# ecmwf/anemoi-core

Measured on AMD Instinct MI355X. Metric: forward nodes*channels/sec on O96 GraphTransformer, higher is better.
Workload: dtype bf16; 1 GPU; AnemoiModelEncProcDec forward, O96 data grid (40320 nodes, 84 vars x 2 steps) -> icosphere res 5 hidden mesh (10242 nodes, 81840 edges), GraphTransformer processor 16 layers x 512 ch x 16 heads, enc 62912 / dec 120960 edges, batch 1; parallelism=single GPU, hip_graph=True, graph_equals_eager=True, graph_segments=1

## Files before the change

### anemoi_core_amd/_lib.py

```python
from __future__ import annotations

import ctypes as C
import os
import threading

ABI_VERSION = 17
LIB_PATH = os.path.join(os.path.dirname(os.path.abspath(__file__)), "lib", "libanemoi_hip.so")

F32, BF16, F16 = 0, 1, 2
ACT_NONE, ACT_GELU = 0, 1
E_INVALID, E_UNSUPPORTED, E_LAUNCH = -1, -2, -3

_p, _i64, _i32, _f = C.c_void_p, C.c_int64, C.c_int32, C.c_float



class LinearPlan(C.Structure):
    _fields_ = [(name, _i32) for name in ("kernel", "tile_m", "tile_n", "pingpong", "stage_k", "mi", "wr", "kg", "stages", "epi", "main_rows",
                                          "tail_rows", "ln_tail_begin")]


SIGNATURES = {
    "anemoi_hip_abi_version": ([], C.c_int),
    "anemoi_hip_last_error": ([], C.c_char_p),
# ... 39 lines not shown
    "anemoi_edge_ln_residual_segment_sum_fwd": ([_p, _i64, _p, _i64, _p, _p, _f, _p, _p, _i64, _p, _i64, _i32, _i32, C.c_int, _p], C.c_int),
    "anemoi_segment_sum_rows": ([_p, _i64, _p, _p, _p, _i64, _i32, _i32, C.c_int, _p], C.c_int),
    "anemoi_gather_add_rows": ([_p, _i64, _p, _i64, _p, _p, _i64, _i32, _i32, C.c_int, _p], C.c_int),
    "anemoi_transpose_pad": ([_p, _i64, _p, _i64, _i32, _i32, _i32, C.c_int, _p], C.c_int),
    "anemoi_glu_fwd": ([_p, _i64, _p, _i64, _i32, _i32, _i32, C.c_int, _p], C.c_int),
    "anemoi_glu_bwd": ([_p, _i64, _p, _i64, _p, _i64, _i32, _i32, _i32, C.c_int, _p], C.c_int),
    "anemoi_gather_rows": ([_p, _i64, _p, _p, _i64, _i32, _i32, C.c_int, _p], C.c_int),
    "anemoi_peer_alloc": ([C.POINTER(_p), _i64, _i32], C.c_int),
    "anemoi_peer_free": ([_p], C.c_int),
    "anemoi_peer_export": ([_p, _p], C.c_int),
    "anemoi_peer_open": ([_p, C.POINTER(_p)], C.c_int),
    "anemoi_peer_close": ([_p], C.c_int),
    "anemoi_gt_chain_rows_per_tile": ([_i32], C.c_int),
    "anemoi_gt_chain2_fwd": ([_p, C.c_int, _p], C.c_int),
    "anemoi_gt_rowchain_fwd": ([_p, C.c_int, _p], C.c_int),
    "anemoi_gt_cluster_chain_fwd": ([_p, C.c_int, _p], C.c_int),
    "anemoi_gt_cluster_chain_workspace_bytes": ([], _i64),
    "anemoi_gnn_edge_chain_fwd": ([_p, _i64, _p, _i64, _p, _p, _i64, _p, _p, _p, _p, _p, _p, _p, _p, _p, _f, _p, _i64, _i32, _i32, C.c_int, _p], C.c_int),
    "anemoi_gnn_mlp_chain_fwd": ([_p, _i64, _i32, _p, _p, _p, _p, _p, _p, _p, _p, _f, _p, _i64, _p, _i64, _i32, _i32, C.c_int, _p], C.c_int),
    "anemoi_gnn_node_chain_segsum_fwd": ([_p, _i64, _p, _i64, _p, _p, _p, _p, _p, _p, _p, _p, _p, _f, _p, _i64, _p, _p, _i32, _p, _i64, _i32, _i32,
                                          C.c_int, _p], C.c_int),
    "anemoi_gnn_node_chain_fwd": ([_p, _i64, _p, _i64, _p, _p, _p, _p, _p, _p, _p, _p, _f, _p, _i64, _p, _p, _i32, _p, _i64, _i32, _i32, C.c_int, _p], C.c_int),
    "anemoi_peer_exchange_rows": ([_p, _i64, _p, _p, _i32, _i32, _i32, _p, _p, _i64, _p], C.c_int),
    "anemoi_window_attention_fwd": ([_p, _i64, _p, _i64, _p, _i64, _p, _i64, _p, _i32, _i32, _i32, _i32, _i32, _f, _f, _p, C.c_int, _p], C.c_int),
    "anemoi_sparse_project_fwd": ([_p, _i64, _i64, _i32, _i64, _i32, _i32, _p, _p, _p, _p, _p, _p, _p, _i64, _i64, _i32, _i32, _i32, C.c_int, C.c_int, _p], C.c_int),
}


EXPERIMENT_SIGNATURES = {
    "anemoi_gt_chain_fwd": ([_p, C.c_int, _p], C.c_int),
# ... 57 lines not shown
```

### anemoi_core_amd/csrc/chain2_core.h

```cpp
#pragma once
#include "chain_core.h"

namespace anemoi {

template <typename T>
__device__ __forceinline__ void gemm128(const unsigned char* abuf, int lane, frag8 (&ring)[2][8], const char* cur, int64_t cs, const char* nxt,
                                        int64_t ns, uint32_t loff, f32x4 (&acc)[3][8], int nq = 8) {
  asm volatile("" : "+v"(lane));
  const int x = lane & 15, ks = lane >> 4;
  const unsigned char* arow = abuf + x * kRowBytes;
  frag8 fa[3];
#pragma unroll
  for (int mi = 0; mi < 3; ++mi) fa[mi] = *reinterpret_cast<const frag8*>(arow + mi * 16 * kRowBytes + ((ks ^ x) << 4));
  const int last = 2 * nq - 1;
#pragma unroll 1
  for (int q = 0; q < nq; ++q) {
    const char* p0 = q < nq - 1 ? cur + (q + 1) * 8192 : nxt;
    const char* p1 = q < nq - 1 ? cur + cs + (q + 1) * 8192 : nxt + ns;
#pragma unroll
    for (int j = 0; j < 2; ++j) {
      const int st = q * 2 + j;
      const int sn = st < last ? st + 1 : last;
      frag8 fn[3];
#pragma unroll
// ... 2 lines not shown
      const gptr_t g0 = uniform_ptr(p0 + j * 4096), g1 = uniform_ptr(p1 + j * 4096);
#pragma unroll
      for (int ni = 0; ni < 8; ++ni) {
#pragma unroll
        for (int mi = 0; mi < 3; ++mi) acc[mi][ni] = cmfma<T>(ring[j][ni], fa[mi], acc[mi][ni]);
        ring[j][ni] = *reinterpret_cast<gfrag_t>((ni < 4 ? g0 : g1) + loff + (ni & 3) * 1024);
        __builtin_amdgcn_sched_barrier(0);
      }
#pragma unroll
      for (int mi = 0; mi < 3; ++mi) fa[mi] = fn[mi];
      __builtin_amdgcn_sched_barrier(0);
    }
  }
}

template <typename T>
__device__ __forceinline__ void gemm64(const unsigned char* abuf, int lane, frag8 (&ring)[2][8], const char* cur, const char* nxt, int64_t ns,
                                       uint32_t loff, f32x4 (&acc)[3][8], int ng = 4) {
  asm volatile("" : "+v"(lane));
  const int x = lane & 15, ks = lane >> 4;
  const unsigned char* arow = abuf + x * kRowBytes;
  frag8 fa[3];
#pragma unroll
  for (int mi = 0; mi < 3; ++mi) fa[mi] = *reinterpret_cast<const frag8*>(arow + mi * 16 * kRowBytes + ((ks ^ x) << 4));
  const int last = ng * 4 - 1;
#pragma unroll 1
  for (int q = 0; q < ng; ++q) {
#pragma unroll
    for (int j = 0; j < 4; ++j) {
      const int st = q * 4 + j;
      const int sn = st < last ? st + 1 : last;
      frag8 fn[3];
#pragma unroll
      for (int mi = 0; mi < 3; ++mi) fn[mi] = *reinterpret_cast<const frag8*>(arow + mi * 16 * kRowBytes + (((sn * 4 + ks) ^ x) << 4));
      __builtin_amdgcn_sched_barrier(0);
      const char* pf = q < ng - 1 ? cur + (q + 1) * 16384 + j * 4096 : (j < 2 ? nxt + j * 4096 : nxt + ns + (j - 2) * 4096);
      const gptr_t g0 = uniform_ptr(pf);
#pragma unroll
      for (int ni = 0; ni < 4; ++ni) {
#pragma unroll
        for (int mi = 0; mi < 3; ++mi) acc[mi][ni] = cmfma<T>(ring[j & 1][(j >> 1) * 4 + ni], fa[mi], acc[mi][ni]);
        ring[j & 1][(j >> 1) * 4 + ni] = *reinterpret_cast<gfrag_t>(g0 + loff + ni * 1024);
        __builtin_amdgcn_sched_barrier(0);
      }
#pragma unroll
      for (int mi = 0; mi < 3; ++mi) fa[mi] = fn[mi];
      __builtin_amdgcn_sched_barrier(0);
    }
  }
}
__device__ __forceinline__ void ring_prologue64(frag8 (&ring)[2][8], const char* f0, uint32_t loff) {
#pragma unroll
  for (int j = 0; j < 4; ++j) {
    const gptr_t g0 = uniform_ptr(f0 + j * 4096);
#pragma unroll
    for (int ni = 0; ni < 4; ++ni) {
      ring[j & 1][(j >> 1) * 4 + ni] = *reinterpret_cast<gfrag_t>(g0 + loff + ni * 1024);
      __builtin_amdgcn_sched_barrier(0);
    }
  }
}
// ... 75 lines not shown
```

### anemoi_core_amd/csrc/chain_core.h

```cpp
#pragma once
#include "common.h"

namespace anemoi {

using frag8 = __attribute__((ext_vector_type(8))) short;
using f32x4 = __attribute__((ext_vector_type(4))) float;

template <typename T>
__device__ __forceinline__ f32x4 cmfma(frag8 a, frag8 b, f32x4 c);
template <>
__device__ __forceinline__ f32x4 cmfma<bf16_t>(frag8 a, frag8 b, f32x4 c) {
  using bf8 = __attribute__((ext_vector_type(8))) __bf16;
  return __builtin_amdgcn_mfma_f32_16x16x32_bf16(__builtin_bit_cast(bf8, a), __builtin_bit_cast(bf8, b), c, 0, 0, 0);
}
template <>
__device__ __forceinline__ f32x4 cmfma<f16_t>(frag8 a, frag8 b, f32x4 c) {
  using h8 = __attribute__((ext_vector_type(8))) _Float16;
  return __builtin_amdgcn_mfma_f32_16x16x32_f16(__builtin_bit_cast(h8, a), __builtin_bit_cast(h8, b), c, 0, 0, 0);
}

using u32x2 = __attribute__((ext_vector_type(2))) unsigned int;
using u32x4 = __attribute__((ext_vector_type(4))) unsigned int;

template <typename T>
// ... 91 lines not shown
#pragma unroll
      for (int mi = 0; mi < NB; ++mi) fa[mi] = fn[mi];
      __builtin_amdgcn_sched_barrier(0);
    }
  }
  if (flip >= 0) __builtin_amdgcn_s_setprio(0);
}

__device__ __forceinline__ void lds_barrier() {
  asm volatile("s_waitcnt lgkmcnt(0)" ::: "memory");
  __builtin_amdgcn_s_barrier();
  asm volatile("" ::: "memory");
}

__device__ __forceinline__ int panel_off(int row, int slot16) { return row * kRowBytes + ((slot16 ^ (row & 15)) << 4); }
template <typename B>
__device__ __forceinline__ B* panel_at(B* buf, int row, int slot16) { return buf + row * kRowBytes + ((slot16 ^ (row & 15)) << 4); }
template <int NI>
constexpr int kWaves = kCh / (16 * NI);

#ifndef ANEMOI_CHAIN2_NT
#define ANEMOI_CHAIN2_NT 1
#endif
__device__ __forceinline__ u32x4 stream_load(const u32x4* p) {
  if constexpr ((ANEMOI_CHAIN2_NT & 1) != 0) return __builtin_nontemporal_load(p);
  else return *p;
}
__device__ __forceinline__ void stream_store(u32x4 v, u32x4* p) {
  if constexpr ((ANEMOI_CHAIN2_NT & 2) != 0) __builtin_nontemporal_store(v, p);
  else if constexpr ((ANEMOI_CHAIN2_NT & 4) != 0) asm volatile("global_store_dwordx4 %0, %1, off sc1" ::"v"(p), "v"(v) : "memory");
  else *p = v;
}
// ... 108 lines not shown
    for (int ni = 0; ni < 4; ++ni)
      *reinterpret_cast<u32x2*>(strip + m * 128 + (((ni * 2 + (lc.g >> 1)) ^ ((m >> 1) & 7)) << 4) + (lc.g & 1) * 8) = pk[mi][ni];
  }
  asm volatile("s_waitcnt lgkmcnt(0)" ::: "memory");
  const int rl = (lc.g << 1) | (lc.x >> 3), sl = lc.x & 7;
#pragma unroll
  for (int it = 0; it < 2 * NB; ++it) {
    const int m = it * 8 + rl;
    const u32x4 v = *reinterpret_cast<const u32x4*>(strip + m * 128 + ((sl ^ ((m >> 1) & 7)) << 4));
    if (m < nr) *reinterpret_cast<u32x4*>(out + (int64_t)m * ld + sl * 8) = v;
  }
  asm volatile("s_waitcnt lgkmcnt(0)" ::: "memory");
}


template <typename T, int NI, bool ROWS>
__device__ __forceinline__ void init_acc(f32x4 (&acc)[3][8], const unsigned char* vec, int col0, const unsigned char* rows, int lane, int w) {
  const LaneCols<NI> lc = lane_cols<NI>(lane, w);
#pragma unroll
  for (int ni = 0; ni < NI; ++ni) {
    float b[4];
    unpack4<T>(*reinterpret_cast<const u32x2*>(vec + (col0 + w * (16 * NI) + ni * 16 + lc.g * 4) * 2), b);
#pragma unroll
    for (int mi = 0; mi < 3; ++mi) {
      if (ROWS) {
        float r[4];
        unpack4<T>(*reinterpret_cast<const u32x2*>(rows + (mi * 16 + lc.x) * kRowBytes + lc.coff[ni]), r);
        acc[mi][ni] = f32x4{b[0] + r[0], b[1] + r[1], b[2] + r[2], b[3] + r[3]};
      } else {
        acc[mi][ni] = f32x4{b[0], b[1], b[2], b[3]};
      }
    }
  }
}

enum class Add { None, Bias, BiasRows };
template <typename T, int NI, Add ADD, bool STATS, bool STORE = true>
__device__ __forceinline__ void round_rows(f32x4 (&acc)[3][8], unsigned char* dst, float* red, int lane, int w, const unsigned char* vec = nullptr, int col0 = 0) {
  const LaneCols<NI> lc = lane_cols<NI>(lane, w);
  u32x2 rb[NI], rr[NI];
  if constexpr (ADD == Add::Bias) {
#pragma unroll
    for (int ni = 0; ni < NI; ++ni) rb[ni] = *reinterpret_cast<const u32x2*>(vec + (col0 + w * (16 * NI) + ni * 16 + lc.g * 4) * 2);
  }
#pragma unroll
  for (int mi = 0; mi < 3; ++mi) {
    unsigned char* drow = dst + (mi * 16 + lc.x) * kRowBytes;
    if constexpr (ADD == Add::BiasRows) {
#pragma unroll
      for (int h = 0; h < NI / 4; ++h) {
#pragma unroll
        for (int ni = 4 * h; ni < 4 * h + 4; ++ni) {
          rb[ni] = *reinterpret_cast<const u32x2*>(vec + (col0 + w * (16 * NI) + ni * 16 + lc.g * 4) * 2);
          rr[ni] = *reinterpret_cast<const u32x2*>(drow + lc.coff[ni]);
        }
        __builtin_amdgcn_sched_barrier(0);
      }
    }
#pragma unroll
    for (int ni = 0; ni < NI; ++ni) {
      float o[4] = {acc[mi][ni][0], acc[mi][ni][1], acc[mi][ni][2], acc[mi][ni][3]};
      if constexpr (ADD != Add::None) {
// ... 28 lines not shown
  const LaneCols<NI> lc = lane_cols<NI>(lane, w);
#pragma unroll
  for (int mi = 0; mi < 3; ++mi) {
    unsigned char* drow = dst + (mi * 16 + lc.x) * kRowBytes;
#pragma unroll
    for (int ni = 0; ni < NI; ++ni) {
      float o[4] = {acc[mi][ni][0], acc[mi][ni][1], acc[mi][ni][2], acc[mi][ni][3]};
      gelu_fast2(o[0], o[1]);
      gelu_fast2(o[2], o[3]);
      *reinterpret_cast<u32x2*>(drow + lc.coff[ni]) = pack4<T>(o);
      if (ni & 1) __builtin_amdgcn_sched_barrier(0);
    }
  }
}

template <typename T, int NI>
__device__ __forceinline__ void normalise_rows(const f32x4 (&acc)[3][8], const float* red, float eps, unsigned char* dst, int lane, int w) {
  const LaneCols<NI> lc = lane_cols<NI>(lane, w);
#pragma unroll
  for (int mi = 0; mi < 3; ++mi) {
    float mu, rstd;
    merge_partials<kWaves<NI>>(red, mi * 16 + lc.x, eps, mu, rstd);
    const float nm = -mu * rstd;
    unsigned char* drow = dst + (mi * 16 + lc.x) * kRowBytes;
#pragma unroll
    for (int ni = 0; ni < NI; ++ni) {
      float o[4];
#pragma unroll
      for (int r = 0; r < 4; ++r) o[r] = fmaf(acc[mi][ni][r], rstd, nm);
      *reinterpret_cast<u32x2*>(drow + lc.coff[ni]) = pack4<T>(o);
    }
  }
}
template <typename T, int NI>
__device__ __forceinline__ void normalise_regs(f32x4 (&acc)[3][8], const float* red, float eps, int lane, int w) {
  const LaneCols<NI> lc = lane_cols<NI>(lane, w);
#pragma unroll
  for (int mi = 0; mi < 3; ++mi) {
    float mu, rstd;
    merge_partials<kWaves<NI>>(red, mi * 16 + lc.x, eps, mu, rstd);
    const float nm = -mu * rstd;
#pragma unroll
    for (int ni = 0; ni < NI; ++ni)
#pragma unroll
      for (int r = 0; r < 4; ++r) acc[mi][ni][r] = fmaf(acc[mi][ni][r], rstd, nm);
  }
}

template <typename T, int NI>
__device__ __forceinline__ void store_staged(const unsigned char* strip, T* out, int64_t ld, int nr, int lane, int w) {
  asm volatile("s_waitcnt lgkmcnt(0)" ::: "memory");
  asm volatile("" : "+v"(lane), "+s"(w));
  constexpr int kLpr = 2 * NI, kRpi = 64 / kLpr;
  const int rl = lane >> (NI == 8 ? 4 : 3), sl = lane & (kLpr - 1);
#pragma unroll
  for (int it = 0; it < kPanel / kRpi; ++it) {
    const int row = it * kRpi + rl;
    const u32x4 v = *reinterpret_cast<const u32x4*>(panel_at(strip, row, w * kLpr + sl));
    if (row < nr) stream_store(v, reinterpret_cast<u32x4*>(out + (int64_t)row * ld + w * (16 * NI) + sl * 8));
  }
}

}
```

### anemoi_core_amd/csrc/gt_rowchain.hip

```cpp
#include "chain2_core.h"

namespace anemoi {

struct RowChainArgs {
  const void* x;   int64_t ld_x;  int k_in;
  const char* we;  int ng;
  const char* wq;  int qc;
  const void* vec;
  float eps;
  void* xout;      int64_t ld_out;
  void* qout;      int64_t ld_q;
  int n_rows, rows_per_tile, n_tiles;
};
constexpr int kRcVecOff = vec_off(8);
constexpr int kRcVecMax = 2560;
constexpr int kRowChainSmem = kRcVecOff + kRcVecMax * 2;
static_assert(kRowChainSmem <= 160 * 1024, "LDS budget");

struct XRows {
  u32x4 v[6];
  __device__ __forceinline__ void request(const void* x, int64_t ld, int k_in, int ng, int r0, int nr, int tid, int es) {
    const int spr = 16 * ng, n = kPanel * spr, kin16 = k_in >> 3;
#pragma unroll
    for (int k = 0; k < 6; ++k) {
      const int i = tid + 512 * k;
      if (k * 512 < n) {
        const int row = min(i / spr, kPanel - 1), slot = i % spr;
        const bool live = row < nr && slot < kin16 && i < n;
        const unsigned char* p = reinterpret_cast<const unsigned char*>(x) + ((int64_t)(r0 + min(row, nr - 1)) * ld + min(slot, kin16 - 1) * 8) * es;
        const u32x4 t = stream_load(reinterpret_cast<const u32x4*>(p));
        v[k] = live ? t : u32x4{0u, 0u, 0u, 0u};
      }
    }
  }
  __device__ __forceinline__ void store(unsigned char* buf, int ng, int tid) {
    const int spr = 16 * ng, n = kPanel * spr;
#pragma unroll
    for (int k = 0; k < 6; ++k) {
      const int i = tid + 512 * k;
      if (i < n) {
        const int row = i / spr, slot = i % spr;
        *reinterpret_cast<u32x4*>(panel_at(buf, row, slot)) = v[k];
      }
    }
  }
};

template <typename T>
__global__ __launch_bounds__(512, 1) void gt_rowchain_kernel(RowChainArgs a) {
  extern __shared__ __attribute__((aligned(16))) unsigned char smem[];
  unsigned char* const bufA = smem;
  unsigned char* const bufB = smem + kBufBytes;
  unsigned char* const bufC = smem + 2 * kBufBytes;
  float* const red = reinterpret_cast<float*>(smem + kRedOff);
  const unsigned char* const vec = smem + kRcVecOff;
  const int tid = threadIdx.x, lane = tid & 63;
  const int w8 = __builtin_amdgcn_readfirstlane(tid >> 6), wq = w8 & 3, grp = w8 >> 2;
  const uint32_t loff = lane * 16;
  const int qc = a.qc, ng = a.ng;
  const int64_t se = (int64_t)ng * 16384;
  const char* const wes = a.we + (int64_t)w8 * se;
// ... 186 lines not shown
  const int w8 = __builtin_amdgcn_readfirstlane(tid >> 6);
  c.wq = w8 & 3;
  c.loff = c.lane * 16;
  c.b0 = (int)blockIdx.x;
  c.grid = (int)gridDim.x;
  if (c.b0 >= a.n_tiles) return;
  c.n = (a.n_tiles - c.b0 + c.grid - 1) / c.grid;
  {
    const int n16 = (512 + 512 * a.qc) / 8;
    if (tid < n16) reinterpret_cast<u32x4*>(smem + kRc2Vec)[tid] = reinterpret_cast<const u32x4*>(a.vec)[tid];
  }
  if (w8 < 4) pipe_role_a<T>(a, c, smem);
  else pipe_role_b<T>(a, c, smem);
}

template <typename T>
static int launch_rowchain(const RowChainArgs& a, hipStream_t st) {
  static PerDeviceOnce once;
  once.run([&] { (void)hipFuncSetAttribute(reinterpret_cast<const void*>(&gt_rowchain_kernel<T>), hipFuncAttributeMaxDynamicSharedMemorySize, kRowChainSmem); });
  int grid = a.n_tiles < 256 ? a.n_tiles : 256;
  if (a.n_tiles > 256) {
    const int rounds = (a.n_tiles + 255) / 256;
    grid = (a.n_tiles + rounds - 1) / rounds;
  }
  if (a.n_tiles > grid && a.k_in <= 256) {
    static PerDeviceOnce once2;
    once2.run([&] { (void)hipFuncSetAttribute(reinterpret_cast<const void*>(&gt_rowchain_pipe_kernel<T>), hipFuncAttributeMaxDynamicSharedMemorySize, kRowChain2Smem); });
    hipLaunchKernelGGL((gt_rowchain_pipe_kernel<T>), dim3(grid), dim3(512), kRowChain2Smem, st, a);
    return check_launch("gt_rowchain_pipe_kernel");
  }
  hipLaunchKernelGGL((gt_rowchain_kernel<T>), dim3(grid), dim3(512), kRowChainSmem, st, a);
  return check_launch("gt_rowchain_kernel");
}

}

using namespace anemoi;

extern "C" int anemoi_gt_rowchain_fwd(const anemoi_gt_rowchain_args_t* p, anemoi_dtype_t dtype, void* stream) {
  ANEMOI_REQUIRE(p != nullptr, "gt_rowchain_fwd: null argument block");
  ANEMOI_REQUIRE(dtype == ANEMOI_BF16 || dtype == ANEMOI_F16, "gt_rowchain_fwd: 16-bit model dtypes only");
  ANEMOI_REQUIRE(p->n_rows >= 0 && p->channels == kCh, "gt_rowchain_fwd: channels=%d (this kernel is built for %d)", p->channels, kCh);
  if (p->n_rows == 0) return ANEMOI_OK;
  ANEMOI_REQUIRE(p->in_features > 0 && p->in_features <= kCh && p->in_features % 8 == 0,
                 "gt_rowchain_fwd: in_features=%d must be a multiple of 8 up to %d (rows move as 16-byte pieces)", p->in_features, kCh);
  ANEMOI_REQUIRE(p->q_out_features > 0 && p->q_out_features % kCh == 0 && p->q_out_features <= 4 * kCh,
                 "gt_rowchain_fwd: q_out_features=%d must be a multiple of %d up to %d", p->q_out_features, kCh, 4 * kCh);
  ANEMOI_REQUIRE(p->x && p->we && p->wq && p->vec && p->q_out, "gt_rowchain_fwd: null operand");
  const auto al16 = [](const void* q) { return (reinterpret_cast<uintptr_t>(q) & 15) == 0; };
  ANEMOI_REQUIRE(al16(p->x) && al16(p->we) && al16(p->wq) && al16(p->vec) && al16(p->x_out) && al16(p->q_out), "gt_rowchain_fwd: operands must be 16-byte aligned");
  ANEMOI_REQUIRE(p->ld_x >= p->in_features && p->ld_x % 8 == 0 && p->ld_q >= p->q_out_features && p->ld_q % 8 == 0 &&
                     (p->x_out == nullptr || (p->ld_out >= kCh && p->ld_out % 8 == 0)),
                 "gt_rowchain_fwd: leading dimensions too small or not multiples of 8 elements");
  RowChainArgs a{};
  a.x = p->x; a.ld_x = p->ld_x; a.k_in = p->in_features;
  a.we = (const char*)p->we; a.ng = (p->in_features + 127) / 128;
  a.wq = (const char*)p->wq; a.qc = p->q_out_features / kCh;
  a.vec = p->vec;
  a.eps = p->ln_eps;
  a.xout = p->x_out; a.ld_out = p->ld_out;
  a.qout = p->q_out; a.ld_q = p->ld_q;
  a.n_rows = p->n_rows;
  a.rows_per_tile = p->rows_per_tile > 0 ? p->rows_per_tile : kPanel;
  ANEMOI_REQUIRE(a.rows_per_tile <= kPanel, "gt_rowchain_fwd: rows_per_tile=%d exceeds the %d-row panel", a.rows_per_tile, kPanel);
  a.n_tiles = (a.n_rows + a.rows_per_tile - 1) / a.rows_per_tile;
  hipStream_t st = as_stream(stream);
  return dtype == ANEMOI_BF16 ? launch_rowchain<bf16_t>(a, st) : launch_rowchain<f16_t>(a, st);
}
```

### anemoi_core_amd/layers/mapper.py

```python
from __future__ import annotations

import os
from typing import Optional

import torch
from torch import Tensor, nn

from .. import ops
from ..distributed import primitives as comm
from ..distributed.partition import (
    build_graph_partition_from_shard_info,
    ensure_edges_are_dst_sorted,
    local_bipartite_graph,
    shard_edges_1hop,
)
from ..distributed.shapes import BipartiteGraphShardInfo, comm_rank, comm_size, get_shard_sizes, model_is_distributed
from .block import GraphConvMapperBlock, GraphTransformerMapperBlock
from .handoff import Carrier, inference_in, plain_layer_norm
from .kernels import PaddedLinear
from .mlp import MLP
from .utils import compute_mlp_hidden_dim, load_layer_kernels
from ..utils.tensors import version


_ROW_CHAIN = os.environ.get("ANEMOI_ROW_CHAIN", "1") != "0"
_ROW_CHAIN_MIN_ROWS = int(os.environ.get("ANEMOI_ROW_CHAIN_MIN_ROWS", "4096"))
_TAIL_PROJ = os.environ.get("ANEMOI_TAIL_PROJ", "1") != "0"
_ROW_CHAIN_GEMM_BAND = tuple(int(v) for v in os.environ.get("ANEMOI_ROW_CHAIN_GEMM_BAND", "16384:262144").split(":"))


class _LocalGraphCache:

    def __init__(self, keep: int = 4):
        self.entries: dict = {}
        self.keep = keep

    def get(self, key, build):
        hit = self.entries.get(key)
        if hit is None:
            hit = build()
            if len(self.entries) >= self.keep:
                self.entries.pop(next(iter(self.entries)))
            self.entries[key] = hit
# ... 61 lines not shown
        self.shard_strategy = shard_strategy
        self.proc = GraphTransformerMapperBlock(
            in_channels=hidden_dim, hidden_dim=compute_mlp_hidden_dim(hidden_dim, mlp_hidden_ratio), out_channels=hidden_dim,
            attn_channels=attn_channels, num_heads=num_heads, edge_dim=edge_dim, qk_norm=qk_norm,
            mlp_implementation=mlp_implementation, layer_kernels=self.layer_factory, shard_strategy=shard_strategy,
            graph_attention_backend=graph_attention_backend, edge_pre_mlp=edge_pre_mlp,
        )
        self.emb_nodes_dst = self.layer_factory.Linear(self.in_channels_dst, self.hidden_dim)
        self._emb_src, self._emb_dst = PaddedLinear(), PaddedLinear()

    def _tail_projection(self):
        return None

    def _row_chain_ok(self, x: Tensor, lin, ln, projs: list) -> bool:
        return (_ROW_CHAIN and x.is_cuda and x.dim() == 2 and x.dtype != torch.float32 and x.shape[0] >= _ROW_CHAIN_MIN_ROWS
                and not (_ROW_CHAIN_GEMM_BAND[0] < x.shape[0] < _ROW_CHAIN_GEMM_BAND[1])
                and self.hidden_dim == ops.CHAIN_CHANNELS and plain_layer_norm(ln) and lin.in_features <= x.shape[1] and lin.bias is not None
                and ops.gt_row_chain_supported(x, sum(p.out_features for p in projs)) and all(p.in_features == ops.CHAIN_CHANNELS for p in projs)
                and inference_in(x, lin, ln, *projs))

    def _row_chain(self, x: Tensor, lin, side: str, want_x: bool):
        blk = self.proc
        ln = blk.layer_norm_attention_src if side == "src" else blk.layer_norm_attention_dest
        projs = [blk.lin_key, blk.lin_value] if side == "src" else [blk.lin_query, blk.lin_self]
        if not self._row_chain_ok(x, lin, ln, projs):
            return None
        params = [lin.weight, lin.bias, ln.weight, ln.bias] + [q for m in projs for q in (m.weight, m.bias)]
        K = x.shape[1]

        def build():
            w = lin.weight if lin.in_features == K else torch.nn.functional.pad(lin.weight, (0, K - lin.in_features))
            wq = torch.cat([m.weight for m in projs], dim=0)
            bq = torch.cat([m.bias if m.bias is not None else m.weight.new_zeros(m.out_features) for m in projs])
            wqg, dq = ops.fold_layer_norm(wq, bq, ln.weight, ln.bias)
            return ops.pack_embedding_frag(w), ops.pack_weight_frag(wqg), torch.cat([lin.bias.float(), dq]).to(x.dtype).contiguous(), wq.shape[0]

        we, wqg, vec, q_out = blk._fused.derived(f"rowchain:{side}:{K}", params, build)
        return ops.gt_row_chain(x, we, wqg, vec, q_out, ln.eps, want_x_out=want_x)

    def _embed(self, padded: PaddedLinear, x: Tensor, lin, side: str, carrier: Optional[Carrier]) -> Tensor:
        ln = self.proc.layer_norm_attention_src if side == "src" else self.proc.layer_norm_attention_dest
        if carrier is not None:
            r = self._row_chain(x, lin, side, want_x=side == "dst" or self.proc.update_src_nodes)
            if r is not None:
                y, proj = r
                return carrier.put(y if y is not None else x.new_empty((x.shape[0], 0)), proj=proj)
            if self.proc._ln_fold_ok(ln, x):
                y, stats = padded.with_row_stats(x, lin)
                return y if stats is None else carrier.put(y, stats=stats)
        return padded(x, lin)

    @comm.scoped_forward
    def forward(self, x, batch_size: int, shard_info: BipartiteGraphShardInfo, edge_attr: Tensor, edge_index: Tensor,
# ... 223 lines not shown
```

### anemoi_core_amd/ops.py

```python
from __future__ import annotations

from dataclasses import dataclass
from typing import NamedTuple, Optional

import os

import torch
from torch import Tensor

from . import _ext, _lib

_DT = {torch.float32: _lib.F32, torch.bfloat16: _lib.BF16, torch.float16: _lib.F16}


def _dt(t: Tensor) -> int:
    try:
        return _DT[t.dtype]
    except KeyError:
        raise ValueError(f"unsupported dtype {t.dtype}; supported: float32, bfloat16, float16") from None


try:
    _raw_stream = torch._C._cuda_getCurrentRawStream
except AttributeError:
# ... 1005 lines not shown
                ("x_out", _p), ("ld_out", _i64), ("q_out", _p), ("ld_q", _i64), ("n_rows", _i32), ("channels", _i32), ("rows_per_tile", _i32)]


def pack_embedding_frag(weight: Tensor) -> Tensor:
    O, K = weight.shape
    pad = (-K) % 128
    w = weight.detach()
    return pack_weight_frag(torch.nn.functional.pad(w, (0, pad)) if pad else w)


def gt_row_chain_supported(x: Tensor, q_out: int) -> bool:
    return (x.is_cuda and x.dim() == 2 and x.dtype in (torch.bfloat16, torch.float16) and 0 < x.shape[1] <= CHAIN_CHANNELS and x.shape[1] % 8 == 0
            and x.stride(1) == 1 and x.stride(0) % 8 == 0 and q_out > 0 and q_out % CHAIN_CHANNELS == 0 and q_out <= 4 * CHAIN_CHANNELS)


def gt_row_chain(x: Tensor, we: Tensor, wqg: Tensor, vec: Tensor, q_out_features: int, ln_eps: float, *, want_x_out: bool = True,
                 rows_per_tile: int = 0):
    _dev(x, we, wqg, vec)
    N, K = x.shape
    dt, D = x.dtype, CHAIN_CHANNELS
    if not gt_row_chain_supported(x, q_out_features):
        raise NotImplementedError(f"gt_row_chain: x {tuple(x.shape)} {dt} / q_out={q_out_features} (16-bit rows of <= {D} columns, a multiple of 8; q_out a multiple of {D})")
    kp = (K + 127) // 128 * 128
    for name, w, numel in (("we", we, D * kp), ("wqg", wqg, q_out_features * D)):
        if w.dim() != 1 or w.numel() != numel or w.dtype != dt or not w.is_contiguous():
            raise ValueError(f"gt_row_chain: {name} must be the contiguous fragment-major image ({numel} x {dt})")
    if vec.dim() != 1 or vec.numel() != D + q_out_features or vec.dtype != dt or not vec.is_contiguous():
        raise ValueError(f"gt_row_chain: vec must be contiguous [{D + q_out_features}] {dt} = cat[be, dq]")
    x_out = torch.empty((N, D), dtype=dt, device=x.device) if want_x_out else None
    q_out = torch.empty((N, q_out_features), dtype=dt, device=x.device)
# ... 271 lines not shown
```

### include/anemoi_hip.h

```cpp
#ifndef ANEMOI_HIP_H
#define ANEMOI_HIP_H

#include <stdint.h>

#ifdef __cplusplus
extern "C" {
#endif

#define ANEMOI_HIP_ABI_VERSION 17

typedef enum { ANEMOI_F32 = 0, ANEMOI_BF16 = 1, ANEMOI_F16 = 2 } anemoi_dtype_t;
typedef enum { ANEMOI_ACT_NONE = 0, ANEMOI_ACT_GELU = 1 } anemoi_act_t;

#define ANEMOI_OK 0
#define ANEMOI_E_INVALID (-1)
#define ANEMOI_E_UNSUPPORTED (-2)
#define ANEMOI_E_LAUNCH (-3)

int anemoi_hip_abi_version(void);
const char* anemoi_hip_last_error(void);

int anemoi_gt_attention_fwd(const void* q, int64_t ldq, const void* k, int64_t ldk, const void* v, int64_t ldv,
                            const void* e, int64_t lde, const int32_t* row, const int32_t* colptr,
                            const void* addend, int64_t ldadd, void* out, int64_t ldo, float* lse,
// ... 175 lines not shown
} anemoi_gt_chain2_args_t;
int anemoi_gt_chain2_fwd(const anemoi_gt_chain2_args_t* args, anemoi_dtype_t dtype, void* stream);
int anemoi_gt_chain_rows_per_tile(int32_t n_rows);

typedef struct anemoi_gt_rowchain_args {
  const void* x;      int64_t ld_x;       int32_t in_features;
  const void* we;
  const void* wq;     int32_t q_out_features;
  const void* vec;
  float ln_eps;
  void* x_out;        int64_t ld_out;
  void* q_out;        int64_t ld_q;
  int32_t n_rows;     int32_t channels;   int32_t rows_per_tile;
} anemoi_gt_rowchain_args_t;
int anemoi_gt_rowchain_fwd(const anemoi_gt_rowchain_args_t* args, anemoi_dtype_t dtype, void* stream);

typedef struct anemoi_gt_cluster_chain_args {
  const void* attn;   int64_t ld_attn;
  const void* x_res;  int64_t ld_x;
  const void* wp;
  const void* w1;     int32_t hidden;
  const void* w2;
  const void* wq;     int32_t q_out_features;
  const void* vec;
  float ln1_eps;      float lnq_eps;
  const void* extra;  int64_t ld_extra;
  void* x_out;        int64_t ld_out;
  void* q_out;        int64_t ld_q;
  void* ln_out;       int64_t ld_ln;
  void* q_out2;       int64_t ld_q2;      int32_t q_split;
// ... 40 lines not shown
```

Measured before the change: 8.635 billion nodes*channels/s.

## Add 96-row tall tile variant of the row-chain embed kernel for narrow inputs

```diff
diff --git a/anemoi_core_amd/_lib.py b/anemoi_core_amd/_lib.py
--- a/anemoi_core_amd/_lib.py
+++ b/anemoi_core_amd/_lib.py
@@ -77,6 +77,7 @@
     "anemoi_gt_chain_rows_per_tile": ([_i32], C.c_int),
     "anemoi_gt_chain2_fwd": ([_p, C.c_int, _p], C.c_int),
     "anemoi_gt_rowchain_fwd": ([_p, C.c_int, _p], C.c_int),
+    "anemoi_gt_rowchain_rows_per_tile": ([_i32, _i32], C.c_int),
     "anemoi_gt_cluster_chain_fwd": ([_p, C.c_int, _p], C.c_int),
     "anemoi_gt_cluster_chain_workspace_bytes": ([], _i64),
     "anemoi_gnn_edge_chain_fwd": ([_p, _i64, _p, _i64, _p, _p, _i64, _p, _p, _p, _p, _p, _p, _p, _p, _p, _f, _p, _i64, _i32, _i32, C.c_int, _p], C.c_int),
diff --git a/anemoi_core_amd/csrc/chain2_core.h b/anemoi_core_amd/csrc/chain2_core.h
--- a/anemoi_core_amd/csrc/chain2_core.h
+++ b/anemoi_core_amd/csrc/chain2_core.h
@@ -40,15 +40,15 @@
   }
 }
 
-template <typename T>
+template <typename T, int NB = 3, int ROWB = kRowBytes>
 __device__ __forceinline__ void gemm64(const unsigned char* abuf, int lane, frag8 (&ring)[2][8], const char* cur, const char* nxt, int64_t ns,
-                                       uint32_t loff, f32x4 (&acc)[3][8], int ng = 4) {
+                                       uint32_t loff, f32x4 (&acc)[NB][8], int ng = 4) {
   asm volatile("" : "+v"(lane));
   const int x = lane & 15, ks = lane >> 4;
-  const unsigned char* arow = abuf + x * kRowBytes;
-  frag8 fa[3];
+  const unsigned char* arow = abuf + x * ROWB;
+  frag8 fa[NB];
 #pragma unroll
-  for (int mi = 0; mi < 3; ++mi) fa[mi] = *reinterpret_cast<const frag8*>(arow + mi * 16 * kRowBytes + ((ks ^ x) << 4));
+  for (int mi = 0; mi < NB; ++mi) fa[mi] = *reinterpret_cast<const frag8*>(arow + mi * 16 * ROWB + ((ks ^ x) << 4));
   const int last = ng * 4 - 1;
 #pragma unroll 1
   for (int q = 0; q < ng; ++q) {
@@ -56,21 +56,21 @@
     for (int j = 0; j < 4; ++j) {
       const int st = q * 4 + j;
       const int sn = st < last ? st + 1 : last;
-      frag8 fn[3];
+      frag8 fn[NB];
 #pragma unroll
-      for (int mi = 0; mi < 3; ++mi) fn[mi] = *reinterpret_cast<const frag8*>(arow + mi * 16 * kRowBytes + (((sn * 4 + ks) ^ x) << 4));
+      for (int mi = 0; mi < NB; ++mi) fn[mi] = *reinterpret_cast<const frag8*>(arow + mi * 16 * ROWB + (((sn * 4 + ks) ^ x) << 4));
       __builtin_amdgcn_sched_barrier(0);
       const char* pf = q < ng - 1 ? cur + (q + 1) * 16384 + j * 4096 : (j < 2 ? nxt + j * 4096 : nxt + ns + (j - 2) * 4096);
       const gptr_t g0 = uniform_ptr(pf);
 #pragma unroll
       for (int ni = 0; ni < 4; ++ni) {
 #pragma unroll
-        for (int mi = 0; mi < 3; ++mi) acc[mi][ni] = cmfma<T>(ring[j & 1][(j >> 1) * 4 + ni], fa[mi], acc[mi][ni]);
+        for (int mi = 0; mi < NB; ++mi) acc[mi][ni] = cmfma<T>(ring[j & 1][(j >> 1) * 4 + ni], fa[mi], acc[mi][ni]);
         ring[j & 1][(j >> 1) * 4 + ni] = *reinterpret_cast<gfrag_t>(g0 + loff + ni * 1024);
         __builtin_amdgcn_sched_barrier(0);
       }
 #pragma unroll
-      for (int mi = 0; mi < 3; ++mi) fa[mi] = fn[mi];
+      for (int mi = 0; mi < NB; ++mi) fa[mi] = fn[mi];
       __builtin_amdgcn_sched_barrier(0);
     }
   }
diff --git a/anemoi_core_amd/csrc/chain_core.h b/anemoi_core_amd/csrc/chain_core.h
--- a/anemoi_core_amd/csrc/chain_core.h
+++ b/anemoi_core_amd/csrc/chain_core.h
@@ -129,8 +129,8 @@
 }
 
 __device__ __forceinline__ int panel_off(int row, int slot16) { return row * kRowBytes + ((slot16 ^ (row & 15)) << 4); }
-template <typename B>
-__device__ __forceinline__ B* panel_at(B* buf, int row, int slot16) { return buf + row * kRowBytes + ((slot16 ^ (row & 15)) << 4); }
+template <int ROWB = kRowBytes, typename B>
+__device__ __forceinline__ B* panel_at(B* buf, int row, int slot16) { return buf + row * ROWB + ((slot16 ^ (row & 15)) << 4); }
 template <int NI>
 constexpr int kWaves = kCh / (16 * NI);
 
@@ -269,18 +269,18 @@
 }
 
 
-template <typename T, int NI, bool ROWS>
-__device__ __forceinline__ void init_acc(f32x4 (&acc)[3][8], const unsigned char* vec, int col0, const unsigned char* rows, int lane, int w) {
+template <typename T, int NI, bool ROWS, int NB = 3, int ROWB = kRowBytes>
+__device__ __forceinline__ void init_acc(f32x4 (&acc)[NB][8], const unsigned char* vec, int col0, const unsigned char* rows, int lane, int w) {
   const LaneCols<NI> lc = lane_cols<NI>(lane, w);
 #pragma unroll
   for (int ni = 0; ni < NI; ++ni) {
     float b[4];
     unpack4<T>(*reinterpret_cast<const u32x2*>(vec + (col0 + w * (16 * NI) + ni * 16 + lc.g * 4) * 2), b);
 #pragma unroll
-    for (int mi = 0; mi < 3; ++mi) {
+    for (int mi = 0; mi < NB; ++mi) {
       if (ROWS) {
         float r[4];
-        unpack4<T>(*reinterpret_cast<const u32x2*>(rows + (mi * 16 + lc.x) * kRowBytes + lc.coff[ni]), r);
+        unpack4<T>(*reinterpret_cast<const u32x2*>(rows + (mi * 16 + lc.x) * ROWB + lc.coff[ni]), r);
         acc[mi][ni] = f32x4{b[0] + r[0], b[1] + r[1], b[2] + r[2], b[3] + r[3]};
       } else {
         acc[mi][ni] = f32x4{b[0], b[1], b[2], b[3]};
@@ -290,8 +290,8 @@
 }
 
 enum class Add { None, Bias, BiasRows };
-template <typename T, int NI, Add ADD, bool STATS, bool STORE = true>
-__device__ __forceinline__ void round_rows(f32x4 (&acc)[3][8], unsigned char* dst, float* red, int lane, int w, const unsigned char* vec = nullptr, int col0 = 0) {
+template <typename T, int NI, Add ADD, bool STATS, bool STORE = true, int NB = 3, int ROWB = kRowBytes>
+__device__ __forceinline__ void round_rows(f32x4 (&acc)[NB][8], unsigned char* dst, float* red, int lane, int w, const unsigned char* vec = nullptr, int col0 = 0) {
   const LaneCols<NI> lc = lane_cols<NI>(lane, w);
   u32x2 rb[NI], rr[NI];
   if constexpr (ADD == Add::Bias) {
@@ -299,8 +299,8 @@
     for (int ni = 0; ni < NI; ++ni) rb[ni] = *reinterpret_cast<const u32x2*>(vec + (col0 + w * (16 * NI) + ni * 16 + lc.g * 4) * 2);
   }
 #pragma unroll
-  for (int mi = 0; mi < 3; ++mi) {
-    unsigned char* drow = dst + (mi * 16 + lc.x) * kRowBytes;
+  for (int mi = 0; mi < NB; ++mi) {
+    unsigned char* drow = dst + (mi * 16 + lc.x) * ROWB;
     if constexpr (ADD == Add::BiasRows) {
 #pragma unroll
       for (int h = 0; h < NI / 4; ++h) {
@@ -359,32 +359,32 @@
   }
 }
 
+template <typename T, int NI, int NB = 3, int ROWB = kRowBytes>
+__device__ __forceinline__ void normalise_rows(const f32x4 (&acc)[NB][8], const float* red, float eps, unsigned char* dst, int lane, int w) {
+  const LaneCols<NI> lc = lane_cols<NI>(lane, w);
+#pragma unroll
+  for (int mi = 0; mi < NB; ++mi) {
+    float mu, rstd;
+    merge_partials<kWaves<NI>>(red, mi * 16 + lc.x, eps, mu, rstd);
+    const float nm = -mu * rstd;
+    unsigned char* drow = dst + (mi * 16 + lc.x) * ROWB;
+#pragma unroll
+    for (int ni = 0; ni < NI; ++ni) {
+      float o[4];
+#pragma unroll
+      for (int r = 0; r < 4; ++r) o[r] = fmaf(acc[mi][ni][r], rstd, nm);
+      *reinterpret_cast<u32x2*>(drow + lc.coff[ni]) = pack4<T>(o);
+    }
+  }
+}
 template <typename T, int NI>
-__device__ __forceinline__ void normalise_rows(const f32x4 (&acc)[3][8], const float* red, float eps, unsigned char* dst, int lane, int w) {
+__device__ __forceinline__ void normalise_regs(f32x4 (&acc)[3][8], const float* red, float eps, int lane, int w) {
   const LaneCols<NI> lc = lane_cols<NI>(lane, w);
 #pragma unroll
   for (int mi = 0; mi < 3; ++mi) {
     float mu, rstd;
     merge_partials<kWaves<NI>>(red, mi * 16 + lc.x, eps, mu, rstd);
     const float nm = -mu * rstd;
-    unsigned char* drow = dst + (mi * 16 + lc.x) * kRowBytes;
-#pragma unroll
-    for (int ni = 0; ni < NI; ++ni) {
-      float o[4];
-#pragma unroll
-      for (int r = 0; r < 4; ++r) o[r] = fmaf(acc[mi][ni][r], rstd, nm);
-      *reinterpret_cast<u32x2*>(drow + lc.coff[ni]) = pack4<T>(o);
-    }
-  }
-}
-template <typename T, int NI>
-__device__ __forceinline__ void normalise_regs(f32x4 (&acc)[3][8], const float* red, float eps, int lane, int w) {
-  const LaneCols<NI> lc = lane_cols<NI>(lane, w);
-#pragma unroll
-  for (int mi = 0; mi < 3; ++mi) {
-    float mu, rstd;
-    merge_partials<kWaves<NI>>(red, mi * 16 + lc.x, eps, mu, rstd);
-    const float nm = -mu * rstd;
 #pragma unroll
     for (int ni = 0; ni < NI; ++ni)
 #pragma unroll
@@ -392,16 +392,16 @@
   }
 }
 
-template <typename T, int NI>
+template <typename T, int NI, int NB = 3, int ROWB = kRowBytes>
 __device__ __forceinline__ void store_staged(const unsigned char* strip, T* out, int64_t ld, int nr, int lane, int w) {
   asm volatile("s_waitcnt lgkmcnt(0)" ::: "memory");
   asm volatile("" : "+v"(lane), "+s"(w));
   constexpr int kLpr = 2 * NI, kRpi = 64 / kLpr;
   const int rl = lane >> (NI == 8 ? 4 : 3), sl = lane & (kLpr - 1);
 #pragma unroll
-  for (int it = 0; it < kPanel / kRpi; ++it) {
+  for (int it = 0; it < 16 * NB / kRpi; ++it) {
     const int row = it * kRpi + rl;
-    const u32x4 v = *reinterpret_cast<const u32x4*>(panel_at(strip, row, w * kLpr + sl));
+    const u32x4 v = *reinterpret_cast<const u32x4*>(panel_at<ROWB>(strip, row, w * kLpr + sl));
     if (row < nr) stream_store(v, reinterpret_cast<u32x4*>(out + (int64_t)row * ld + w * (16 * NI) + sl * 8));
   }
 }
diff --git a/anemoi_core_amd/csrc/gt_rowchain.hip b/anemoi_core_amd/csrc/gt_rowchain.hip
--- a/anemoi_core_amd/csrc/gt_rowchain.hip
+++ b/anemoi_core_amd/csrc/gt_rowchain.hip
@@ -17,15 +17,16 @@
 constexpr int kRowChainSmem = kRcVecOff + kRcVecMax * 2;
 static_assert(kRowChainSmem <= 160 * 1024, "LDS budget");
 
-struct XRows {
+template <int ROWS = kPanel, int ROWB = kRowBytes, bool POW2 = false>
+struct XRowsT {
   u32x4 v[6];
   __device__ __forceinline__ void request(const void* x, int64_t ld, int k_in, int ng, int r0, int nr, int tid, int es) {
-    const int spr = 16 * ng, n = kPanel * spr, kin16 = k_in >> 3;
+    const int spr = 16 * ng, n = ROWS * spr, kin16 = k_in >> 3;
 #pragma unroll
     for (int k = 0; k < 6; ++k) {
       const int i = tid + 512 * k;
       if (k * 512 < n) {
-        const int row = min(i / spr, kPanel - 1), slot = i % spr;
+        const int row = min(POW2 ? i >> (3 + ng) : i / spr, ROWS - 1), slot = POW2 ? i & (spr - 1) : i % spr;
         const bool live = row < nr && slot < kin16 && i < n;
         const unsigned char* p = reinterpret_cast<const unsigned char*>(x) + ((int64_t)(r0 + min(row, nr - 1)) * ld + min(slot, kin16 - 1) * 8) * es;
         const u32x4 t = stream_load(reinterpret_cast<const u32x4*>(p));
@@ -34,17 +35,18 @@
     }
   }
   __device__ __forceinline__ void store(unsigned char* buf, int ng, int tid) {
-    const int spr = 16 * ng, n = kPanel * spr;
+    const int spr = 16 * ng, n = ROWS * spr;
 #pragma unroll
     for (int k = 0; k < 6; ++k) {
       const int i = tid + 512 * k;
       if (i < n) {
-        const int row = i / spr, slot = i % spr;
-        *reinterpret_cast<u32x4*>(panel_at(buf, row, slot)) = v[k];
+        const int row = POW2 ? i >> (3 + ng) : i / spr, slot = POW2 ? i & (spr - 1) : i % spr;
+        *reinterpret_cast<u32x4*>(panel_at<ROWB>(buf, row, slot)) = v[k];
       }
     }
   }
 };
+using XRows = XRowsT<>;
 
 template <typename T>
 __global__ __launch_bounds__(512, 1) void gt_rowchain_kernel(RowChainArgs a) {
@@ -261,10 +263,109 @@
   else pipe_role_b<T>(a, c, smem);
 }
 
+constexpr int kTallRows = 96, kTallBands = kTallRows / 16;
+constexpr int kTallXRow = 512;
+constexpr int kTallMaxIn = kTallXRow / 2;
+constexpr int kTallXBytes = kTallRows * kTallXRow;
+constexpr int kTallYOff = kTallXBytes;
+constexpr int kTallRedOff = kTallYOff + kTallRows * kRowBytes;
+constexpr int kTallVecOff = kTallRedOff + kTallRows * 8 * 2 * 4;
+constexpr int kTallSmem = kTallVecOff + kRcVecMax * 2;
+constexpr int kTallStrip = kTallXBytes / 8;
+static_assert(kTallSmem == 155 * 1024 && kTallSmem <= 160 * 1024, "LDS budget: 48 + 96 + 6 + 5 KiB");
+static_assert(kTallStrip == kPanel * 128, "a wave stages half a panel (three row bands) of its 64 columns at a time");
+
+template <typename T>
+__global__ __launch_bounds__(512, 1) void gt_rowchain_tall_kernel(RowChainArgs a) {
+  extern __shared__ __attribute__((aligned(16))) unsigned char smem[];
+  unsigned char* const bufX = smem;
+  unsigned char* const bufY = smem + kTallYOff;
+  float* const red = reinterpret_cast<float*>(smem + kTallRedOff);
+  const unsigned char* const vec = smem + kTallVecOff;
+  const int tid = threadIdx.x, lane = tid & 63;
+  const int w8 = __builtin_amdgcn_readfirstlane(tid >> 6);
+  const uint32_t loff = lane * 16;
+  const int qc = a.qc, ng = a.ng;
+  const char* const wes = a.we + (int64_t)w8 * ((int64_t)ng * 16384);
+  auto wqs = [&](int k) { return a.wq + (int64_t)(8 * k + w8) * kSlab; };
+  unsigned char* const strip = bufX + w8 * kTallStrip;
+  int tile = blockIdx.x;
+  if (tile >= a.n_tiles) return;
+  frag8 ring[2][8];
+  f32x4 acc[kTallBands][8];
+  XRowsT<kTallRows, kTallXRow, true> xr;
+  {
+    const int r0 = tile * a.rows_per_tile;
+    xr.request(a.x, a.ld_x, a.k_in, ng, r0, min(a.rows_per_tile, a.n_rows - r0), tid, (int)sizeof(T));
+    const int n16 = (512 + 512 * qc) / 8;
+    u32x4 vv = reinterpret_cast<const u32x4*>(a.vec)[min(tid, n16 - 1)];
+    ring_prologue64(ring, wes, loff);
+    xr.store(bufX, ng, tid);
+    if (tid < n16) reinterpret_cast<u32x4*>(smem + kTallVecOff)[tid] = vv;
+    lds_barrier();
+  }
+  for (;;) {
+    const int r0 = tile * a.rows_per_tile;
+    const int nr = min(a.rows_per_tile, a.n_rows - r0);
+    const int tile_next = tile + (int)gridDim.x;
+    const bool more = tile_next < a.n_tiles;
+#pragma unroll
+    for (int mi = 0; mi < kTallBands; ++mi)
+#pragma unroll
+      for (int ni = 0; ni < 4; ++ni) acc[mi][ni] = f32x4{0.f, 0.f, 0.f, 0.f};
+    gemm64<T, kTallBands, kTallXRow>(bufX, lane, ring, wes, wqs(0), 8192, loff, acc, ng);
+    round_rows<T, 4, Add::Bias, true, true, kTallBands>(acc, bufY, red, lane, w8, vec);
+    if (a.xout != nullptr) store_staged<T, 4, kTallBands>(bufY, (T*)a.xout + (int64_t)r0 * a.ld_out, a.ld_out, nr, lane, w8);
+    lds_barrier();
+    normalise_rows<T, 4, kTallBands>(acc, red, a.eps, bufY, lane, w8);
+    lds_barrier();
+    for (int k = 0; k < qc; ++k) {
+      const bool last = k + 1 == qc;
+      if (last && more) {
+        const int rn = tile_next * a.rows_per_tile;
+        int t = tid;
+        asm volatile("" : "+v"(t));
+        xr.request(a.x, a.ld_x, a.k_in, ng, rn, min(a.rows_per_tile, a.n_rows - rn), t, (int)sizeof(T));
+      }
+      init_acc<T, 4, false, kTallBands>(acc, vec, 512 + 512 * k, nullptr, lane, w8);
+      gemm64<T, kTallBands>(bufY, lane, ring, wqs(k), last ? wes : wqs(k + 1), 8192, loff, acc);
+      T* const out = (T*)a.qout + (int64_t)r0 * a.ld_q + k * kCh + w8 * 64;
+#pragma unroll
+      for (int h = 0; h < 2; ++h) {
+        u32x2 pk[3][4];
+#pragma unroll
+        for (int mi = 0; mi < 3; ++mi)
+#pragma unroll
+          for (int ni = 0; ni < 4; ++ni) {
+            const float o[4] = {acc[3 * h + mi][ni][0], acc[3 * h + mi][ni][1], acc[3 * h + mi][ni][2], acc[3 * h + mi][ni][3]};
+            pk[mi][ni] = pack4<T>(o);
+          }
+        store_block_via_strip<T, 3>(pk, strip, out + (int64_t)(kPanel * h) * a.ld_q, a.ld_q, nr - kPanel * h, lane, w8);
+      }
+    }
+    if (!more) break;
+    lds_barrier();
+    tile = tile_next;
+    {
+      int t = tid;
+      asm volatile("" : "+v"(t));
+      xr.store(bufX, ng, t);
+    }
+    lds_barrier();
+  }
+}
+
 template <typename T>
 static int launch_rowchain(const RowChainArgs& a, hipStream_t st) {
   static PerDeviceOnce once;
   once.run([&] { (void)hipFuncSetAttribute(reinterpret_cast<const void*>(&gt_rowchain_kernel<T>), hipFuncAttributeMaxDynamicSharedMemorySize, kRowChainSmem); });
+  if (a.rows_per_tile > kPanel) {
+    static PerDeviceOnce once3;
+    once3.run([&] { (void)hipFuncSetAttribute(reinterpret_cast<const void*>(&gt_rowchain_tall_kernel<T>), hipFuncAttributeMaxDynamicSharedMemorySize, kTallSmem); });
+    const int rounds = (a.n_tiles + 255) / 256;
+    hipLaunchKernelGGL((gt_rowchain_tall_kernel<T>), dim3((a.n_tiles + rounds - 1) / rounds), dim3(512), kTallSmem, st, a);
+    return check_launch("gt_rowchain_tall_kernel");
+  }
   int grid = a.n_tiles < 256 ? a.n_tiles : 256;
   if (a.n_tiles > 256) {
     const int rounds = (a.n_tiles + 255) / 256;
@@ -283,6 +384,10 @@
 }
 
 using namespace anemoi;
+
+extern "C" int anemoi_gt_rowchain_rows_per_tile(int32_t n_rows, int32_t in_features) {
+  return in_features <= kTallMaxIn && n_rows > 256 * kPanel ? kTallRows : kPanel;
+}
 
 extern "C" int anemoi_gt_rowchain_fwd(const anemoi_gt_rowchain_args_t* p, anemoi_dtype_t dtype, void* stream) {
   ANEMOI_REQUIRE(p != nullptr, "gt_rowchain_fwd: null argument block");
@@ -308,8 +413,10 @@
   a.xout = p->x_out; a.ld_out = p->ld_out;
   a.qout = p->q_out; a.ld_q = p->ld_q;
   a.n_rows = p->n_rows;
-  a.rows_per_tile = p->rows_per_tile > 0 ? p->rows_per_tile : kPanel;
-  ANEMOI_REQUIRE(a.rows_per_tile <= kPanel, "gt_rowchain_fwd: rows_per_tile=%d exceeds the %d-row panel", a.rows_per_tile, kPanel);
+  ANEMOI_REQUIRE(p->rows_per_tile >= 0 && p->rows_per_tile <= kTallRows, "gt_rowchain_fwd: rows_per_tile=%d (0: the library chooses; at most %d)", p->rows_per_tile, kTallRows);
+  a.rows_per_tile = p->rows_per_tile > 0 ? p->rows_per_tile : anemoi_gt_rowchain_rows_per_tile(p->n_rows, p->in_features);
+  ANEMOI_REQUIRE(a.rows_per_tile <= kPanel || p->in_features <= kTallMaxIn, "gt_rowchain_fwd: rows_per_tile=%d needs in_features=%d <= %d (panels above %d rows)",
+                 a.rows_per_tile, p->in_features, kTallMaxIn, kPanel);
   a.n_tiles = (a.n_rows + a.rows_per_tile - 1) / a.rows_per_tile;
   hipStream_t st = as_stream(stream);
   return dtype == ANEMOI_BF16 ? launch_rowchain<bf16_t>(a, st) : launch_rowchain<f16_t>(a, st);
diff --git a/anemoi_core_amd/layers/mapper.py b/anemoi_core_amd/layers/mapper.py
--- a/anemoi_core_amd/layers/mapper.py
+++ b/anemoi_core_amd/layers/mapper.py
@@ -27,6 +27,22 @@
 _ROW_CHAIN_MIN_ROWS = int(os.environ.get("ANEMOI_ROW_CHAIN_MIN_ROWS", "4096"))
 _TAIL_PROJ = os.environ.get("ANEMOI_TAIL_PROJ", "1") != "0"
 _ROW_CHAIN_GEMM_BAND = tuple(int(v) for v in os.environ.get("ANEMOI_ROW_CHAIN_GEMM_BAND", "16384:262144").split(":"))
+_ROW_CHAIN_TALL = os.environ.get("ANEMOI_ROW_CHAIN_TALL", "1") != "0"
+_ROW_CHAIN_TALL_MIN_ROWS = int(os.environ.get("ANEMOI_ROW_CHAIN_TALL_MIN_ROWS", "-1"))
+_ROW_CHAIN_TALL_MAX_IN = 256
+
+
+def _row_chain_rows_per_tile(n_rows: int, in_features: int) -> int:
+    if not _ROW_CHAIN_TALL:
+        return 48
+    if _ROW_CHAIN_TALL_MIN_ROWS >= 0:
+        return 96 if in_features <= _ROW_CHAIN_TALL_MAX_IN and n_rows >= _ROW_CHAIN_TALL_MIN_ROWS else 48
+    return 0
+
+
+def _row_chain_is_tall(n_rows: int, in_features: int) -> bool:
+    rpt = _row_chain_rows_per_tile(n_rows, in_features)
+    return (rpt or ops.gt_row_chain_rows_per_tile(n_rows, in_features)) > 48
 
 
 class _LocalGraphCache:
@@ -118,7 +134,7 @@
 
     def _row_chain_ok(self, x: Tensor, lin, ln, projs: list) -> bool:
         return (_ROW_CHAIN and x.is_cuda and x.dim() == 2 and x.dtype != torch.float32 and x.shape[0] >= _ROW_CHAIN_MIN_ROWS
-                and not (_ROW_CHAIN_GEMM_BAND[0] < x.shape[0] < _ROW_CHAIN_GEMM_BAND[1])
+                and (not (_ROW_CHAIN_GEMM_BAND[0] < x.shape[0] < _ROW_CHAIN_GEMM_BAND[1]) or _row_chain_is_tall(x.shape[0], x.shape[1]))
                 and self.hidden_dim == ops.CHAIN_CHANNELS and plain_layer_norm(ln) and lin.in_features <= x.shape[1] and lin.bias is not None
                 and ops.gt_row_chain_supported(x, sum(p.out_features for p in projs)) and all(p.in_features == ops.CHAIN_CHANNELS for p in projs)
                 and inference_in(x, lin, ln, *projs))
@@ -140,7 +156,7 @@
             return ops.pack_embedding_frag(w), ops.pack_weight_frag(wqg), torch.cat([lin.bias.float(), dq]).to(x.dtype).contiguous(), wq.shape[0]
 
         we, wqg, vec, q_out = blk._fused.derived(f"rowchain:{side}:{K}", params, build)
-        return ops.gt_row_chain(x, we, wqg, vec, q_out, ln.eps, want_x_out=want_x)
+        return ops.gt_row_chain(x, we, wqg, vec, q_out, ln.eps, want_x_out=want_x, rows_per_tile=_row_chain_rows_per_tile(x.shape[0], K))
 
     def _embed(self, padded: PaddedLinear, x: Tensor, lin, side: str, carrier: Optional[Carrier]) -> Tensor:
         ln = self.proc.layer_norm_attention_src if side == "src" else self.proc.layer_norm_attention_dest
diff --git a/anemoi_core_amd/ops.py b/anemoi_core_amd/ops.py
--- a/anemoi_core_amd/ops.py
+++ b/anemoi_core_amd/ops.py
@@ -1043,6 +1043,10 @@
             and x.stride(1) == 1 and x.stride(0) % 8 == 0 and q_out > 0 and q_out % CHAIN_CHANNELS == 0 and q_out <= 4 * CHAIN_CHANNELS)
 
 
+def gt_row_chain_rows_per_tile(n_rows: int, in_features: int) -> int:
+    return int(_lib.load().anemoi_gt_rowchain_rows_per_tile(int(n_rows), int(in_features)))
+
+
 def gt_row_chain(x: Tensor, we: Tensor, wqg: Tensor, vec: Tensor, q_out_features: int, ln_eps: float, *, want_x_out: bool = True,
                  rows_per_tile: int = 0):
     _dev(x, we, wqg, vec)
diff --git a/include/anemoi_hip.h b/include/anemoi_hip.h
--- a/include/anemoi_hip.h
+++ b/include/anemoi_hip.h
@@ -213,6 +213,7 @@
   int32_t n_rows;     int32_t channels;   int32_t rows_per_tile;
 } anemoi_gt_rowchain_args_t;
 int anemoi_gt_rowchain_fwd(const anemoi_gt_rowchain_args_t* args, anemoi_dtype_t dtype, void* stream);
+int anemoi_gt_rowchain_rows_per_tile(int32_t n_rows, int32_t in_features);
 
 typedef struct anemoi_gt_cluster_chain_args {
   const void* attn;   int64_t ld_attn;
```

Measured after the change: 8.721 billion nodes*channels/s (median of 6 runs). About the same (+1.0%).
